# dkarpushkin/rs-pathtracing

Hardware: AMD Instinct MI355X
Metric: Msamples/sec cornell_box 1920x1080x256spp at 1/2/4/8 MI355X; RMS pixel delta (higher is better)
Workload: dtype f64; 1 GPU; cornell_box.json 1920x1080 256spp depth 8; config=c2, width=1920, height=1080, spp=256, depth=8, seed=1, parallelism=single GPU, wf_slots=2

## Files before the change

### __graft_entry__.py

```python
import importlib.util
import os
import subprocess
import sys
from pathlib import Path

ROOT = Path(__file__).resolve().parent


def load_package():
    if "rs_pathtracing_amd" in sys.modules:
        return sys.modules["rs_pathtracing_amd"]
    pkg = ROOT / "rs-pathtracing_amd"
    spec = importlib.util.spec_from_file_location("rs_pathtracing_amd", pkg / "__init__.py",
                                                  submodule_search_locations=[str(pkg)])
    mod = importlib.util.module_from_spec(spec)
    sys.modules["rs_pathtracing_amd"] = mod
    spec.loader.exec_module(mod)
    return mod


def build() -> None:
    env = dict(os.environ, PYTORCH_ROCM_ARCH="gfx950")
    jobs = str(min(8, os.cpu_count() or 1))
    subprocess.run(["make", "-j", jobs, "-C", str(ROOT / "rs-pathtracing_amd")], check=True, env=env)
    subprocess.run(["make", "-C", str(ROOT / "oracle")], check=True, env=env)
    subprocess.run(["make", "-j", jobs, "-C", str(ROOT / "tests" / "native")], check=True, env=env)
    subprocess.run(["make", "-C", str(ROOT / "tests" / "march_clip")], check=True, env=env)
    subprocess.run(["make", "-C", str(ROOT / "tools"), "pt_render"], check=True, env=env)
    pt = load_package()
    pt.lib()
    print("built", pt.LIB_PATH, "-", pt.version())


def smoke() -> None:
    import numpy as np

    pt = load_package()
    sys.path.insert(0, str(ROOT / "oracle"))
    import oracle

    text = (ROOT / "scenes" / "cornell_box.json").read_text()
    scene = pt.Scene.from_json(text, seed=1)
    r = pt.HipRenderer(scene, device=0, depth=8)
    w, h, spp = 48, 27, 2
    img = r.render(scene.camera(), pt.ImageParams(w, h), spp, seed=1)
    ref = oracle.Scene(text, seed=1).render(w, h, spp, 8, 1)
    rms = np.sqrt(np.mean((img - ref) ** 2, axis=0))
    exact = float(np.mean(np.all(img == ref, axis=1)))
    print("smoke: %dx%d@%dspp mean=%s rms=%s exact_pixels=%.4f" % (w, h, spp, img.mean(0), rms, exact))
    assert np.all(rms <= 1e-4), rms
# ... 8 lines not shown
```

### rs-pathtracing_amd/csrc/pt_api.cpp

```cpp
#include <hip/hip_runtime.h>

#include <algorithm>
#include <atomic>
#include <chrono>
#include <cmath>
#include <cstddef>
#include <cstring>
#include <new>
#include <string>
#include <thread>
#include <type_traits>
#include <vector>

#include "../../include/rs_pathtracing.h"
#include "pt_accel.hpp"
#include "pt_adaptive.hpp"
#include "pt_aov.hpp"
#include "pt_denoise.hpp"
#include "pt_kernel.hpp"
#include "pt_plan.hpp"
#include "pt_scene.hpp"
#include "pt_temporal.hpp"
#include "pt_tiles.hpp"
#include "pt_variance.hpp"
// ... 332 lines not shown
    const std::vector<DQGrid> qbuf = pack_qnodes(acc);
    hipError_t err = hipSetDevice(device);
    const DNodeC *nodes = upload(err, acc.cnodes, fault);
    const int32_t *leaf = upload(err, acc.leaf, fault);
    const int32_t *lin = upload(err, acc.lin, fault);
    const int32_t *march = upload(err, acc.march, fault);
    const DBox *boxes = upload(err, acc.boxes, fault);
    const DQGrid *qnodes = qbuf.empty() ? nullptr : upload(err, qbuf, fault);
    StagedAccel a{};
    view_set_accel(a, acc, nodes, qnodes, leaf, lin, march, boxes);
    if (err != hipSuccess) {
        free_staged(device, a);
        return hip_fail(err, "uploading the acceleration structure");
    }
    *out = a;
    return PT_OK;
}

int commit_accel(GpuShare &g, StagedAccel &a) {
    HIP_TRY(hipSetDevice(g.device));
    HIP_TRY(hipDeviceSynchronize());
    StagedAccel old = g.ds.view;
    view_set_accel(g.ds.view, a);
    a = StagedAccel{};
    free_staged(g.device, old);
    return PT_OK;
}

int init_share(GpuShare &g, int device, const Scene &S, const Accel &acc, const std::vector<DShape> &hs,
               const std::vector<DMaterial> &hm) {
    g.device = device;
    HIP_TRY(hipSetDevice(device));
    hipError_t err = hipStreamCreateWithFlags(&g.stream, hipStreamNonBlocking);
    const DShape *shapes = upload(err, hs);
    const DMaterial *mats = upload(err, hm);
    const bool tex = !S.textures.empty();
    const DTexture *textures = tex ? upload(err, S.textures) : nullptr;
    const DPerlin *perlins = tex ? upload(err, S.perlins) : nullptr;
    const DImage *images = tex ? upload(err, S.images) : nullptr;
    const uint8_t *pixels = tex ? upload(err, S.pixels) : nullptr;
    view_set_scene(g.ds.view, S, shapes, mats, textures, perlins, images, pixels);
    if (err == hipSuccess) err = hipEventCreateWithFlags(&g.shard_ev, hipEventDisableTiming);
    if (err == hipSuccess) err = hipMalloc((void **)&g.ds.view.guard, 4 * sizeof(unsigned long long));
    if (err == hipSuccess) err = hipMemset(g.ds.view.guard, 0, 4 * sizeof(unsigned long long));
    if (err != hipSuccess) return hip_fail(err, "uploading the scene");
    StagedAccel a{};
// ... 286 lines not shown
        r->fault_accel_alloc = (int)value;
        return PT_OK;
    }
    for (auto &g : r->gpus) {
        Tuning t = g.ws.tune;
        if (!tuning_set(&t, name, value))
            return fail(PT_ERR_INVALID, std::string("unknown option or value out of range: ") + name + " = " +
                                            std::to_string((long long)value));
        HIP_TRY(hipSetDevice(g.device));
        HIP_TRY(hipDeviceSynchronize());
        g.ws.tune = t;
        g.ds.view.diag = t.diag;
    }
    return PT_OK;
}

int pt_renderer_get_option(const pt_renderer *r, const char *name, int64_t *value) {
    if (!r || !name || !value) return fail(PT_ERR_INVALID, "null argument");
    if (!std::strcmp(name, "bvh_nodes")) {
        *value = r->gpus[0].ds.view.nnodes;
        return PT_OK;
    }
    if (ran_get(r->gpus[0].ws.ran, name, value)) return PT_OK;
    if (!tuning_get(r->gpus[0].ws.tune, name, value)) return fail(PT_ERR_INVALID, std::string("unknown option: ") + name);
    return PT_OK;
}

const char *pt_option_name(int index) {
    return index >= 0 && index < KNOB_COUNT ? KNOBS[index].name : nullptr;
}

int pt_renderer_peer_access(const pt_renderer *r, int *pairs, int *enabled) {
    if (!r) return fail(PT_ERR_INVALID, "null renderer");
    if (pairs) *pairs = r->peer_pairs;
    if (enabled) *enabled = r->peer_enabled;
    return PT_OK;
}

int pt_renderer_num_devices(const pt_renderer *r) { return r ? (int)r->gpus.size() : fail(PT_ERR_INVALID, "null renderer"); }

void pt_renderer_destroy(pt_renderer *r) {
    if (!r) return;
    if (r->started) (void)pt_render_stop(r);
    join_feeder(r);
    (void)sync_all(r);
    release_bands(r);
// ... 831 lines not shown
```

### rs-pathtracing_amd/csrc/pt_device.hpp

```cpp
#pragma once
#include <hip/hip_runtime.h>

#include <cstdint>

#include "pt_lprof.hpp"
#include "pt_march.hpp"
#include "pt_tiles.hpp"
#include "pt_torus.hpp"
#include "pt_types.hpp"

namespace pt {
namespace dev {

__device__ __forceinline__ bool stopped(const int *flag) {
    return flag && __hip_atomic_load(flag, __ATOMIC_RELAXED, __HIP_MEMORY_SCOPE_SYSTEM) != 0;
}

struct V3 {
    double x, y, z;
};
PT_HD V3 v3(double x, double y, double z) { return V3{x, y, z}; }
PT_HD V3 add(V3 a, V3 b) { return v3(a.x + b.x, a.y + b.y, a.z + b.z); }
PT_HD V3 sub(V3 a, V3 b) { return v3(a.x - b.x, a.y - b.y, a.z - b.z); }
PT_HD double dot(V3 a, V3 b) { return a.x * b.x + a.y * b.y + a.z * b.z; }
PT_HD V3 scale(V3 a, double s) { return v3(a.x * s, a.y * s, a.z * s); }
PT_HD V3 divs(V3 a, double s) { return v3(a.x / s, a.y / s, a.z / s); }
PT_HD V3 neg(V3 a) { return v3(-a.x, -a.y, -a.z); }
// ... 263 lines not shown

template <bool STATS>
PT_HD void bvh_leaf_test(const Scene &sc, const Ray &r, bool axis_ok, int first, int count, bool direct,
                         double min_t, double &best, int &who, Ctr *ct) {
    for (int k = 0; k < count; k++) {
        int i = direct ? first : sc.leaf[first + k];
        PT_LP(BVH_LEAF);
        double t;
        const DShape &S = sc.shapes[i];
        bool h;
        if (axis_ok && S.axis) {
            if (STATS) ct->c[C_TEST_SPHERE]++;
            h = sphere_axis_t(S.inv, r.o, r.d, min_t, best, &t);
        } else {
            h = shape_test<STATS, march::F_ANY, false>(S, r, min_t, best, &t, ct);
        }
        if (h && (t < best || i > who)) {
            best = t;
            who = i;
        }
    }
}

template <bool STATS = false, bool EXT = false, bool FMA_SLAB = false, bool QN = false, int PART = 3>
PT_HD void closest_nomarch(const Scene &sc, const Ray &r, V3 inv, double min_t, double *best_t, int *who_out,
                           Ctr *ct = nullptr, bool any = false) {
    double best = *best_t;
    int who = *who_out;
    double g_pz = 0.0, g_dz = 1.0, g_ox = 0.0, g_oy = 0.0, g_dx = 0.0, g_dy = 0.0;
    for (int k = 0; k < ((PART & 1) ? sc.nlin : 0); k++) {
        if (any && wave_all(who >= 0)) break;
        const int entry = uniform_index(uniform_load(&sc.lin[k]));
        const int i = entry & LIN_ID_MASK;
        const DShape s = uniform_shape(&sc.shapes[i]);
        PT_LP(ULIST_SHAPE);
        if (s.type == RECTANGLE) {
            if (STATS) ct->c[C_TEST_RECT]++;
            const double *m = s.inv;
            if (!(entry & LIN_GROUPED)) {
                g_pz = r.o.x * m[8] + r.o.y * m[9] + r.o.z * m[10];
                g_dz = r.d.x * m[8] + r.d.y * m[9] + r.d.z * m[10];
                g_ox = r.o.x * m[0] + r.o.y * m[1] + r.o.z * m[2];
                g_oy = r.o.x * m[4] + r.o.y * m[5] + r.o.z * m[6];
                g_dx = r.d.x * m[0] + r.d.y * m[1] + r.d.z * m[2];
                g_dy = r.d.x * m[4] + r.d.y * m[5] + r.d.z * m[6];
            }
            const double oz = g_pz + m[11];
            const double tt = -oz / g_dz;
            bool h = !(tt < min_t || tt > best);
            if (h) {
                PT_LP(RECT_ROWS);
                const double px = (g_ox + m[3]) + g_dx * tt, py = (g_oy + m[7]) + g_dy * tt;
                h = !(px < s.p[0] || px > s.p[2] || py < s.p[1] || py > s.p[3]);
            }
            if (h && (tt < best || i > who)) {
                best = tt;
                who = i;
            }
            continue;
        }
        if (s.type == CUBE || s.type == SPHERE) {
            if (STATS) ct->c[C_NODE_SLABS]++;
// ... 658 lines not shown
```

### rs-pathtracing_amd/csrc/pt_kernel.hip

```cpp
#include <hip/hip_runtime.h>

#include "pt_device.hpp"
#include "pt_kernel.hpp"

#include <cstdlib>
#include <cstring>

namespace pt {

using dev::Ray;
using dev::V3;

template <int NW, int WAVES, int FK = march::F_ANY>
__global__ __launch_bounds__(256, WAVES) void render_tiles(dev::Scene sc, FrameParams P, double *__restrict__ out) {
    if (P.stop) {
        __shared__ int halt;
        if (threadIdx.x == 0) {
            halt = dev::stopped(P.stop);
            if (halt) dev::note_stop(sc.guard, false);
        }
        __syncthreads();
        if (halt) return;
    }
    const uint32_t ti = P.tile_begin + blockIdx.x;
// ... 169 lines not shown
    if (l == (uint32_t)__ffsll((long long)bal) - 1) {
        atomicAdd(&acc[0], (unsigned long long)pt.trace);
        atomicAdd(&acc[1], (unsigned long long)pt.march);
        atomicAdd(&acc[2], (unsigned long long)pt.select);
        atomicAdd(&acc[3], (unsigned long long)(pt.finish + pt.scatter + pt.restart));
        atomicAdd(&acc[7], (unsigned long long)pt.finish);
        atomicAdd(&acc[8], (unsigned long long)pt.scatter);
        atomicAdd(&acc[9], (unsigned long long)pt.restart);
    }
    atomicAdd(&acc[4], (unsigned long long)pt.passes);
    atomicAdd(&acc[5], (unsigned long long)pt.march_passes);
    atomicMax(&acc[6], (unsigned long long)pt.passes);
}

#define PT_DISPATCH_NW(depth, CALL)                                        \
    switch (builds::stack_words(depth)) {                                  \
    case 4: { constexpr int NW = 4; CALL; } break;                         \
    case 8: { constexpr int NW = 8; CALL; } break;                         \
    case 16: { constexpr int NW = 16; CALL; } break;                       \
    default: { constexpr int NW = 32; CALL; } break;                       \
    }

hipError_t launch_render_wave(const dev::Scene &sc, const FrameParams &P, double *out, hipStream_t st,
                              WaveWorkspace *ws, const builds::Choice &ch, const uint32_t *tiles);

hipError_t launch_render(const DeviceScene &s, const FrameParams &P, double *out, hipStream_t st, WaveWorkspace &ws,
                         const uint32_t *tiles) {
    ws.ran = builds::Ran{};
    if (P.tile_count == 0) return hipSuccess;
    ws.refusal[0] = 0;
    builds::Inputs in{};
    in.ext = s.view.ext != 0;
    in.fkind = s.fkind;
    in.nnodes = s.view.nnodes;
    in.nmarch = s.view.nmarch;
    in.has_qnodes = s.view.qnodes != nullptr;
    in.scene_diag = s.view.diag;
    in.depth = P.depth;
    in.samples = (uint64_t)P.tile_count * TILE * TILE * P.spp;
    in.window = P.s_begin > 0 || (P.s_end && P.s_end < P.spp) || tiles != nullptr;
    in.window_empty = P.s_begin >= (P.s_end ? P.s_end : P.spp);
    in.wave_diag_on = PT_WAVE_DIAG && ws.diag;
    in.diag_buffer = ws.diag != nullptr;
    in.tune = ws.tune;
    const builds::Choice ch = builds::choose(in);
    if (ch.engine == builds::REFUSE) return hipErrorInvalidValue;
    if (ch.engine == builds::WAVE) return launch_render_wave(s.view, P, out, st, &ws, ch, tiles);
    if (tiles) return hipErrorInvalidValue;
    hipError_t e0 = timer_begin(ws.timer, st, K_MEGA);
    if (e0 != hipSuccess) return e0;
    bool launched = false;
#define X(NW, WAVES, FK)                                                             \
    if (ch.mega.is(NW, WAVES, FK)) {                                                 \
        render_tiles<NW, WAVES, FK><<<P.tile_count, 256, 0, st>>>(s.view, P, out);   \
        ws.ran.engine = builds::MEGA;                                                \
        ws.ran.mega = builds::key(NW, WAVES, FK);                                    \
        launched = true;                                                             \
    }
    PT_MEGA_BUILDS(X)
#undef X
    if (!launched) return hipErrorInvalidValue;
    e0 = hipGetLastError();
    if (e0 != hipSuccess) return e0;
    return timer_end(ws.timer, st);
}

hipError_t launch_unshard(const double *g, uint32_t width, uint32_t height, uint32_t world, double *frame,
                          hipStream_t st, uint32_t y0, uint32_t y1) {
    uint32_t tiles_x = (width + TILE - 1) / TILE, tiles_y = (height + TILE - 1) / TILE;
    uint32_t total = tiles_x * tiles_y;
// ... 96 lines not shown
```

### rs-pathtracing_amd/csrc/pt_kernel.hpp

```cpp
#pragma once
#include <hip/hip_runtime.h>

#include "../../include/rs_pathtracing.h"
#include "pt_builds.hpp"
#include "pt_types.hpp"

namespace pt {

struct DeviceScene {
    dev::Scene view = {};
    int nshapes = 0;
    int fkind = 0;
};

enum KernelKind : int { K_BOUNCE = 0, K_MARCH = 1, K_SELECT = 2, K_REDUCE = 3, K_MEGA = 4, K_UNWIND = 5, K_WALK = 6, K_KINDS = 7 };
struct KernelTimer;
KernelTimer *timer_new();
void timer_free(KernelTimer *t);
hipError_t timer_begin(KernelTimer *t, hipStream_t st, int kind);
hipError_t timer_end(KernelTimer *t, hipStream_t st);
hipError_t timer_collect(KernelTimer *t, double *ms, uint32_t *launches);

#ifndef PT_WAVE_DIAG
#define PT_WAVE_DIAG 0
#endif

struct WaveWorkspace {
    Tuning tune;
    void *base = nullptr;
    size_t bytes = 0;
    unsigned long long *diag = nullptr;
    KernelTimer *timer = nullptr;
    static constexpr int MAX_SLOTS = WF_MAX_SLOTS;
    hipStream_t side[MAX_SLOTS - 1] = {};
    hipEvent_t fork = nullptr, join[MAX_SLOTS - 1] = {}, reduced = nullptr;
    hipEvent_t done = nullptr;
    bool used = false;
    void *args_host = nullptr, *args_dev = nullptr;
    size_t args_bytes = 0;
    hipEvent_t args_ev = nullptr;
    bool args_pending = false;
    int device = -1;
    char refusal[320] = {};
    builds::Ran ran;
};
void wave_workspace_free(WaveWorkspace *ws);

hipError_t launch_render(const DeviceScene &s, const FrameParams &P, double *out, hipStream_t st, WaveWorkspace &ws,
                         const uint32_t *tiles = nullptr);
hipError_t launch_unshard(const double *gathered, uint32_t width, uint32_t height, uint32_t world, double *frame,
                          hipStream_t st, uint32_t y0 = 0, uint32_t y1 = ~0u);
hipError_t launch_encode_rgba8(const double *rgb, size_t p0, size_t p1, uint8_t *rgba, hipStream_t st);
hipError_t launch_closest_hit(const DeviceScene &s, const double *rays, size_t n, double min_t, double max_t,
                              pt_hit *out, hipStream_t st);
hipError_t launch_ray_color(const DeviceScene &s, const double *rays, uint64_t *states, size_t n, uint32_t depth,
                            double s11, double *out, hipStream_t st);
hipError_t launch_trace_pixels(const DeviceScene &s, const FrameParams &P, const uint32_t *pixels, size_t n,
                               double *out, hipStream_t st);

hipError_t launch_count_work(const DeviceScene &s, const FrameParams &P, const uint32_t *pixels, size_t n,
                             unsigned long long *ctr, hipStream_t st);

hipError_t launch_march_probe(const double *jobs, size_t n, double *t, int32_t *status, uint32_t *iters,
                              hipStream_t st);
hipError_t launch_render_timed(const DeviceScene &s, const FrameParams &P, double *out, unsigned long long *acc,
                               hipStream_t st);

}
```

### rs-pathtracing_amd/csrc/pt_lprof.hpp

```cpp
#pragma once
#include <hip/hip_runtime.h>

#ifdef PT_MARCH_REGIONS
namespace pt {
namespace mreg {
enum { R_ITER, R_POLY, R_PREFIX, R_HALVE, R_ADV, R_LIT, R_REFILL, R_TOTAL, R_N };
enum { P_iters, P_lin_init, P_lit_adds, P_advance_loops, P_evals, P_sir_inside, P_lin_fail_zero, P_lin_fail_q,
       P_lin_fail_tie, P_lin_fail_zone, P_N };
constexpr int G_N = 2 * R_N + 2 * P_N;
__device__ unsigned long long g_acc[G_N];
__shared__ unsigned long long t0[4][R_N], acc[4][R_N], accl[4][R_N], n0[4][R_N], pw[4][P_N], pl[4][P_N];
__device__ __forceinline__ unsigned long long now() {
    __builtin_amdgcn_sched_barrier(0);
    const unsigned long long t = __builtin_amdgcn_s_memtime();
    __builtin_amdgcn_sched_barrier(0);
    return t;
}
__device__ __forceinline__ bool leader() {
    const uint32_t lane = __builtin_amdgcn_mbcnt_hi(~0u, __builtin_amdgcn_mbcnt_lo(~0u, 0u));
    return lane == (uint32_t)__builtin_ctzll(__ballot(1));
}
__device__ __forceinline__ void begin(int r) {
    const unsigned long long m = __ballot(1);
    if (leader()) {
// ... 115 lines not shown
    const uint32_t lane = __builtin_amdgcn_mbcnt_hi(~0u, __builtin_amdgcn_mbcnt_lo(~0u, 0u));
    if (lane == (uint32_t)__builtin_ctzll(m)) {
        atomicAdd(&s_pass[k], 1ull);
        atomicAdd(&s_lanes[k], (unsigned long long)__popcll(m));
    }
}
__device__ __forceinline__ void begin_kernel() {
    if (threadIdx.x < N_POINTS) s_pass[threadIdx.x] = s_lanes[threadIdx.x] = 0;
    __syncthreads();
}
__device__ __forceinline__ void end_kernel() {
    __syncthreads();
    if (threadIdx.x < N_POINTS) {
        atomicAdd(&g_counts[threadIdx.x], s_pass[threadIdx.x]);
        atomicAdd(&g_counts[N_POINTS + threadIdx.x], s_lanes[threadIdx.x]);
    }
}
}
}
#endif
#if defined(PT_LANE_PROF) && defined(__HIP_DEVICE_COMPILE__)
#define PT_LP(k) pt::lprof::hit(pt::lprof::k)
#define PT_LP_BEGIN() pt::lprof::begin_kernel()
#define PT_LP_END() pt::lprof::end_kernel()
#else
#define PT_LP(k) ((void)0)
#define PT_LP_BEGIN() ((void)0)
#define PT_LP_END() ((void)0)
#endif
```

### rs-pathtracing_amd/csrc/pt_wave.hip

```cpp
#include <hip/hip_runtime.h>

#include <cstdio>
#include <cstdlib>
#include <cstring>
#include <vector>

#include "pt_lprof.hpp"

#include "pt_device.hpp"
#include "pt_kernel.hpp"
#include "pt_plan.hpp"

namespace pt {

using dev::MemStack;
using dev::Ray;
using dev::V3;

constexpr uint32_t WHO_MASK = (1u << 25) - 1u;
__host__ __device__ __forceinline__ uint32_t pack_who(int who, uint32_t count) {
    return (uint32_t)(who + 1) | (count << 25);
}
__host__ __device__ __forceinline__ int unpack_who(uint32_t w) { return (int)(w & WHO_MASK) - 1; }

// ... 9 lines not shown
    }
    __host__ __device__ uint32_t *d4(uint32_t k) const {
        return (uint32_t *)(base + (size_t)(k / BLK) * BLK_BYTES + 8 * 8 * BLK) + (k % BLK);
    }
    __host__ __device__ double &t(uint32_t k) const { return d8(k)[T * BLK]; }
    __host__ __device__ uint32_t &who(uint32_t k) const { return d4(k)[WHO * BLK]; }
};

struct WfView {
    PathSoA in, out;
    uint32_t *ids;
    double *att;
    double *leaf;
    uint8_t *status;
    uint32_t *list, *mq;
    double2 *jo;
    uint32_t *cnt;
    double *acc;
    uint32_t cap;
    uint32_t npix;
    uint32_t s0, ns;
    uint32_t tile0;
    const uint32_t *tile_map;
};

struct alignas(64) WfArgs {
    dev::Scene sc;
    FrameParams P;
    WfView v;
};

template <class T>
__device__ __forceinline__ const T &kargs(const T *p) {
    typedef const __attribute__((address_space(4))) T *cptr;
    cptr q = (cptr)p;
    asm volatile("" : "+s"(q));
    return *(const T *)q;
}

__device__ __forceinline__ uint32_t lane_id() {
    return __builtin_amdgcn_mbcnt_hi(~0u, __builtin_amdgcn_mbcnt_lo(~0u, 0u));
}

constexpr int UB = 4;
template <bool EXT>
__device__ __forceinline__ V3 unwind_mem(const dev::Scene &sc, MemStack &stk, V3 c) {
// ... 110 lines not shown
    PT_LP_BEGIN();
#define PT_BSTAMP(k)                                                \
    if (DIAG) {                                                     \
        __builtin_amdgcn_s_waitcnt(0);                              \
        const unsigned long long n_ = __builtin_amdgcn_s_memtime(); \
        dsec[k] += n_ - tst;                                        \
        tst = n_;                                                   \
    }
    for (uint32_t base = blockIdx.x * blockDim.x; base < count; base += stride) {
        if (DIAG) tst = __builtin_amdgcn_s_memtime();
        const WfArgs &a = kargs(A);
        const dev::Scene &sc = a.sc;
        const FrameParams &P = a.P;
        const WfView &v = a.v;
        const uint32_t i = base + threadIdx.x;
        bool live = i < count;
        uint32_t id = 0;
        Ray ray;
        dev::Rng rng{0};
        uint32_t depth = 0;
        MemStack stk{v.ids, (size_t)v.cap, 0, nullptr};
        int who = -1;
        double best = 0.0;
        if (live) {
            if (FIRST) {
                id = i;
                uint32_t x, y, sl, pl;
                slot_pixel(P, v, id, &x, &y, &sl, &pl);
                if (x >= P.width || y >= P.height || sl >= v.ns) {
                    live = false;
                } else {
                    rng.s = dev::sample_key(P.seed, (uint64_t)x + (uint64_t)y * P.width, v.s0 + sl);
                    ray = dev::camera_ray(P, x, y, rng);
                    depth = P.depth;
                    stk.base = v.ids + id;
                    if (EXT) stk.vb = v.att + id;
                }
            } else {
                const uint32_t p = v.list[i];
                PT_BSTAMP(0)
                uint32_t count;
                load_path(v.in, p, &id, &ray, &rng.s, P.depth + 1u - (uint32_t)it, &depth, &count, &who, &best);
                stk.base = v.ids + id;
                stk.n = DEEP ? (int)*deep_count(v, P.depth, id) : (int)count;
                if (EXT) stk.vb = v.att + id;
                PT_BSTAMP(1)
            }
        }
        bool need_march = false, long_job = false;
        V3 jo_o = dev::v3(0.0, 0.0, 0.0), jo_d = jo_o;
        double jo_st = 0.0, jo_en = 0.0;
        if (live) {
            PT_LP(LIVE);
            if (!FIRST) {
                V3 leaf;
                const bool ended = dev::shade<false, FK, EXT>(kargs(A).sc, who, best, ray, depth, stk, rng, P.s11, &leaf);
                PT_BSTAMP(2)
                if (ended) {
                    PT_LP(ENDED);
                    end_path(v, id, stk, leaf);
                    live = false;
                    PT_BSTAMP(3)
                }
            }
        }
        if (live && SPLIT) {
            best = __builtin_inf();
            who = -1;
        } else if (live) {
            PT_LP(TRACE);
            const V3 inv = dev::v3(1.0 / ray.d.x, 1.0 / ray.d.y, 1.0 / ray.d.z);
            best = __builtin_inf();
            who = -1;
            const bool any = depth == 0;
            dev::closest_nomarch<false, EXT, BIGBVH>(kargs(A).sc, ray, inv, T_MIN, &best, &who, nullptr, any);
            PT_BSTAMP(4)
            for (int k = 0; k < sc.nmarch && !need_march && !(any && who >= 0); k++) {
                const int s = dev::uniform_index(dev::uniform_load(&sc.march[k]));
                const DBox bx = dev::uniform_box(&sc.boxes[s]);
                if (!dev::slab(bx.lo, bx.hi, ray, inv, T_MIN, best)) continue;
                PT_LP(PRE_SLAB);
                const DShape S = dev::uniform_shape(&sc.shapes[s]);
                jo_o = dev::xf_point(S.inv, ray.o);
                jo_d = dev::xf_vector(S.inv, ray.d);
                need_march = march::shape_bound_k<FK>(dev::shape_params(S), jo_o.x, jo_o.y, jo_o.z, jo_d.x, jo_d.y,
                                                      jo_d.z, &jo_st, &jo_en);
                need_march = need_march && march::clip_to_best(best, S.p[0], &jo_st, &jo_en);
            }
            PT_BSTAMP(5)
            if (!need_march && dev::shade_decided(who, depth)) {
                if (any) PT_LP(ANY_END);
                else PT_LP(MISS_END);
                end_path(v, id, stk, dev::decided_leaf(who, ray));
                live = false;
            }
        }
        const uint32_t wbase = base + (threadIdx.x & ~63u);
        const uint64_t keep = __ballot(live);
        const uint32_t k = wbase + (uint32_t)__popcll(keep & ((1ull << (threadIdx.x & 63)) - 1ull));
        if (i < count && (threadIdx.x & 63) >= (uint32_t)__popcll(keep)) v.status[i] = 0u;
// ... 6 lines not shown
            __builtin_nontemporal_store((d2v){jo_d.y, jo_d.z}, j + 2);
            __builtin_nontemporal_store((d2v){jo_st, jo_en}, j + 3);
            const march::FParams F = dev::shape_params(dev::uniform_shape(&sc.shapes[dev::uniform_index(
                dev::uniform_load(&sc.march[0]))]));
            const V3 o = jo_o, d = jo_d;
            const double st = jo_st, en = jo_en;
            long_job = march::shape_f_k<FK>(F, o.x + d.x * st, o.y + d.y * st, o.z + d.z * st) < 0.0;
            const double dt = (en - st) * (1.0 / WF_PREDICT);
#pragma unroll
            for (int q = 0; q < WF_PREDICT; q++) {
                const double tq = st + dt * (q + 0.5);
                long_job = long_job || march::shape_f_k<FK>(F, o.x + d.x * tq, o.y + d.y * tq, o.z + d.z * tq) < 0.0;
            }
        }
        if (i < count) PT_LP(STORE);
        if (i < count && live) {
            store_path(v.out, k, id, ray, best, who, rng.s, DEEP ? 0u : (uint32_t)stk.n);
            if (DEEP) *deep_count(v, P.depth, id) = (uint32_t)stk.n;
            v.status[k] = live ? (need_march ? (long_job ? 7u : 3u) : 1u) : 0u;
        }
        PT_BSTAMP(6)
    }
#undef PT_BSTAMP
    PT_LP_END();
    if (DIAG && (threadIdx.x & 63) == 0)
        for (int k = 0; k < 7; k++) atomicAdd(&diag[36 + k], dsec[k]);
}


__device__ __forceinline__ void cp_bits(uint4 q, uint32_t *live, uint32_t *march, uint32_t *lng) {
    const uint32_t w[4] = {q.x, q.y, q.z, q.w};
    uint32_t l = 0, m = 0, g = 0;
#pragma unroll
    for (int k = 0; k < 4; k++) {
        l += __popc(w[k] & 0x01010101u);
        m += __popc(w[k] & 0x02020202u);
        g += __popc(w[k] & 0x04040404u);
    }
    *live = l;
    *march = m;
    *lng = g;
}

__device__ __forceinline__ uint32_t block_exscan(uint32_t x, uint32_t *total, uint32_t *lds ) {
    const uint32_t lane = threadIdx.x & 63, wv = threadIdx.x >> 6;
    uint32_t inc = x;
#pragma unroll
// ... 543 lines not shown
    if (ws->args_host) (void)hipHostFree(ws->args_host);
    if (ws->args_dev) (void)hipFree(ws->args_dev);
    ws->args_host = ws->args_dev = nullptr;
    ws->args_bytes = 0;
    ws->args_pending = false;
}

static void release_streams(WaveWorkspace *ws) {
    free_args(ws);
    for (int k = 0; k < WaveWorkspace::MAX_SLOTS - 1; k++) {
        if (ws->side[k]) (void)hipStreamDestroy(ws->side[k]);
        if (ws->join[k]) (void)hipEventDestroy(ws->join[k]);
        ws->side[k] = nullptr;
        ws->join[k] = nullptr;
    }
    if (ws->fork) (void)hipEventDestroy(ws->fork);
    if (ws->reduced) (void)hipEventDestroy(ws->reduced);
    if (ws->done) (void)hipEventDestroy(ws->done);
    if (ws->args_ev) (void)hipEventDestroy(ws->args_ev);
    ws->fork = ws->reduced = ws->done = ws->args_ev = nullptr;
    ws->used = false;
}

void wave_workspace_free(WaveWorkspace *ws) {
    release_streams(ws);
    timer_free(ws->timer);
    ws->timer = nullptr;
    if (ws->diag) (void)hipFree(ws->diag);
    ws->diag = nullptr;
    if (ws->base) (void)hipFree(ws->base);
    ws->base = nullptr;
    ws->bytes = 0;
}

static hipError_t reserve_args(WaveWorkspace *ws, size_t bytes) {
    hipError_t e;
    if (ws->args_pending) {
        if ((e = hipEventSynchronize(ws->args_ev)) != hipSuccess) return e;
        ws->args_pending = false;
    }
    if (bytes <= ws->args_bytes) return hipSuccess;
    if (ws->used && (e = hipEventSynchronize(ws->done)) != hipSuccess) return e;
    free_args(ws);
    if (bytes < ((size_t)64 << 10)) bytes = (size_t)64 << 10;
    if ((e = hipHostMalloc(&ws->args_host, bytes, hipHostMallocDefault)) != hipSuccess) {
        ws->args_host = nullptr;
        return e;
    }
    if ((e = hipMalloc(&ws->args_dev, bytes)) != hipSuccess) {
        ws->args_dev = nullptr;
        free_args(ws);
        return e;
// ... 92 lines not shown
    if (unwound)
        wf_reduce<EXT, true><<<blocks, 256, 0, st>>>(A, first, last, out);
    else
        wf_reduce<EXT, false><<<blocks, 256, 0, st>>>(A, first, last, out);
    return hipSuccess;
}

template <class F>
static hipError_t timed(KernelTimer *t, hipStream_t st, int kind, F launch) {
    hipError_t e = timer_begin(t, st, kind);
    if (e != hipSuccess) return e;
    if ((e = launch()) != hipSuccess) return e;
    if ((e = hipGetLastError()) != hipSuccess) return e;
    return timer_end(t, st);
}

static hipError_t ensure_streams(WaveWorkspace *ws, int slots) {
    int dev = 0;
    hipError_t e = hipGetDevice(&dev);
    if (e != hipSuccess) return e;
    if (ws->device != dev) {
        if (ws->used && ws->done && (e = hipEventSynchronize(ws->done)) != hipSuccess) return e;
        release_streams(ws);
        ws->device = dev;
    }
    if (!ws->fork && (e = hipEventCreateWithFlags(&ws->fork, hipEventDisableTiming)) != hipSuccess) return e;
    if (!ws->done && (e = hipEventCreateWithFlags(&ws->done, hipEventDisableTiming)) != hipSuccess) return e;
    if (!ws->reduced && (e = hipEventCreateWithFlags(&ws->reduced, hipEventDisableTiming)) != hipSuccess) return e;
    if (!ws->args_ev && (e = hipEventCreateWithFlags(&ws->args_ev, hipEventDisableTiming)) != hipSuccess) return e;
    for (int k = 0; k < slots - 1; k++) {
        if (!ws->side[k] && (e = hipStreamCreateWithFlags(&ws->side[k], hipStreamNonBlocking)) != hipSuccess) return e;
        if (!ws->join[k] && (e = hipEventCreateWithFlags(&ws->join[k], hipEventDisableTiming)) != hipSuccess) return e;
    }
    return hipSuccess;
}

struct Slot {
    WfView v;
    uint32_t *cp_blk;
    PathSoA set[2];
};

static hipStream_t slot_stream(const WaveWorkspace *ws, hipStream_t st, int j) { return j == 0 ? st : ws->side[j - 1]; }

hipError_t launch_render_wave(const dev::Scene &sc, const FrameParams &P0, double *out, hipStream_t st,
                              WaveWorkspace *ws, const builds::Choice &bc, const uint32_t *tiles) {
    if (P0.tile_count == 0 || P0.spp == 0) return hipSuccess;
    const Tuning &tu = ws->tune;
    plan::Input in;
    in.ntiles = P0.tile_count;
    in.s_begin = P0.s_begin;
    in.s_end = P0.s_end ? P0.s_end : P0.spp;
    in.spp = P0.spp;
    in.depth = P0.depth;
    in.progressive = P0.stop != nullptr;
    in.textured = sc.tex != nullptr;
    in.presel = bc.presel;
    in.wf_paths = tu.wf_paths;
    in.wf_slots = tu.wf_slots;
    in.wf_min_chunks = tu.wf_min_chunks;
    in.avail_bytes = plan::MEM_UNKNOWN;
    size_t free_b = 0, total_b = 0, hard_bytes = plan::MEM_UNKNOWN;
    if (hipMemGetInfo(&free_b, &total_b) == hipSuccess) {
        hard_bytes = free_b + ws->bytes;
        in.avail_bytes = hard_bytes > plan::RESERVE_BYTES ? hard_bytes - plan::RESERVE_BYTES : 0;
    }
    if (!plan::depth_ok(P0.depth)) {
        snprintf(ws->refusal, sizeof ws->refusal, "depth %u is above the largest supported depth, %u", P0.depth,
                 plan::MAX_DEPTH);
        return hipErrorInvalidValue;
    }
    const plan::Plan pl = plan::make_plan_fit(&in, hard_bytes);
    if (!plan::fits_device(pl, hard_bytes)) {
        snprintf(ws->refusal, sizeof ws->refusal,
                 "the wavefront workspace does not fit the device: depth %u, %s scene, %u paths per chunk on %d "
                 "stream(s) need %zu bytes, %zu bytes available",
                 P0.depth, in.textured ? "textured" : "untextured", pl.cap, pl.slots, pl.bytes, hard_bytes);
        return hipErrorOutOfMemory;
    }
    const plan::Layout &L = pl.lay;
    const std::vector<plan::Chunk> chunk_list = plan::chunk_list(in, pl);
    const int slots = pl.slots, iters = pl.iters;
    const uint32_t s_begin = in.s_begin, s_end = in.s_end;

    hipError_t e = ensure_streams(ws, slots);
    if (e != hipSuccess) return e;
    if (ws->used && (e = hipStreamWaitEvent(st, ws->done, 0)) != hipSuccess) return e;
    if ((e = reserve(ws, pl.bytes)) != hipSuccess) return e;
    Slot sl[WaveWorkspace::MAX_SLOTS];
    for (int k = 0; k < slots; k++) {
        char *slot = (char *)ws->base + (size_t)k * L.slot_stride;
        auto at = [&](plan::Region r) { return L.size[r] ? (void *)(slot + L.off[r]) : nullptr; };
        sl[k].set[0] = PathSoA{(char *)at(plan::R_SET0), pl.cap};
        sl[k].set[1] = PathSoA{(char *)at(plan::R_SET1), pl.cap};
        sl[k].cp_blk = (uint32_t *)at(plan::R_CP_BLK);
        WfView &v = sl[k].v;
        v.ids = (uint32_t *)at(plan::R_IDS);
        v.leaf = (double *)at(plan::R_LEAF);
        v.list = (uint32_t *)at(plan::R_LIST);
        v.mq = (uint32_t *)at(plan::R_MQ);
        v.status = (uint8_t *)at(plan::R_STATUS);
        v.cnt = (uint32_t *)at(plan::R_CNT);
        v.att = (double *)at(plan::R_ATT);
        v.jo = (double2 *)at(plan::R_JO);
        v.acc = (double *)((char *)ws->base + L.acc);
        v.cap = pl.cap;
    }

    const uint32_t march_slice = (uint32_t)tu.wf_march_slice;
    unsigned long long *const bounce_diag = bc.bounce.diag ? ws->diag : nullptr;
    unsigned long long *const march_diag = bc.march.diag ? ws->diag : nullptr;
    const size_t nargs = chunk_list.size() * 2;
    const size_t list_off = (nargs * sizeof(WfArgs) + 15) & ~(size_t)15;
    const size_t args_bytes = tiles ? list_off + (size_t)P0.tile_count * sizeof(uint32_t) : nargs * sizeof(WfArgs);
    if ((e = reserve_args(ws, args_bytes)) != hipSuccess) return e;
    WfArgs *ah = (WfArgs *)ws->args_host, *ad = (WfArgs *)ws->args_dev;
    const uint32_t *tile_map = nullptr;
    if (tiles) {
        memcpy((char *)ws->args_host + list_off, tiles, (size_t)P0.tile_count * sizeof(uint32_t));
        tile_map = (const uint32_t *)((char *)ws->args_dev + list_off);
    }
    for (size_t ci = 0; ci < chunk_list.size(); ci++) {
        const plan::Chunk &ch = chunk_list[ci];
        const int j = ch.slot;
        WfView v = sl[j].v;
        v.tile0 = P0.tile_begin + ch.g0;
        v.tile_map = tile_map;
        v.npix = ch.gt * TILE * TILE;
        v.s0 = ch.s0;
        v.ns = ch.ns;
        for (int h = 0; h < 2; h++) {
            v.in = sl[j].set[h];
            v.out = sl[j].set[h ^ 1];
            ah[2 * ci + h] = WfArgs{sc, P0, v};
        }
    }
    if ((e = hipMemcpyAsync(ad, ah, args_bytes, hipMemcpyHostToDevice, st)) != hipSuccess) return e;
    if ((e = hipEventRecord(ws->args_ev, st)) != hipSuccess) return e;
    ws->args_pending = true;
    if (slots > 1) {
        if ((e = hipEventRecord(ws->fork, st)) != hipSuccess) return e;
        for (int k = 0; k < slots - 1; k++)
            if ((e = hipStreamWaitEvent(ws->side[k], ws->fork, 0)) != hipSuccess) return e;
    }
    for (size_t r0 = 0; r0 < chunk_list.size();) {
        size_t r1 = r0;
        while (r1 < chunk_list.size() && chunk_list[r1].step == chunk_list[r0].step) r1++;
        for (size_t c = r0; c < r1; c++) {
            const int j = chunk_list[c].slot;
            const hipStream_t cs = slot_stream(ws, st, j);
// ... 105 lines not shown
```

Before: 2322 Msamples/s.

## Cull unreachable shapes for primary rays using per-8x8-block frustum masks

Adds a per-frame table, built by a small kernel, that holds a 64-bit mask for each 8x8 pixel block. Each bit says whether a list shape or march shape's bounding box can intersect that block's sub-frustum. The first-bounce kernel reads the mask with a wave-uniform load and skips shapes outside the frustum in both the linear list and the march loop. Grouped-rectangle caching is made aware of skipped entries. The table is cached by camera key and accel generation, at the cost of an extra kernel launch when the camera changes and some added branching in the primary-ray loop.

```diff
diff --git a/__graft_entry__.py b/__graft_entry__.py
--- a/__graft_entry__.py
+++ b/__graft_entry__.py
@@ -26,6 +26,7 @@
     subprocess.run(["make", "-C", str(ROOT / "oracle")], check=True, env=env)
     subprocess.run(["make", "-j", jobs, "-C", str(ROOT / "tests" / "native")], check=True, env=env)
     subprocess.run(["make", "-C", str(ROOT / "tests" / "march_clip")], check=True, env=env)
+    subprocess.run(["make", "-C", str(ROOT / "tests" / "first_cull")], check=True, env=env)
     subprocess.run(["make", "-C", str(ROOT / "tools"), "pt_render"], check=True, env=env)
     pt = load_package()
     pt.lib()
diff --git a/rs-pathtracing_amd/csrc/pt_api.cpp b/rs-pathtracing_amd/csrc/pt_api.cpp
--- a/rs-pathtracing_amd/csrc/pt_api.cpp
+++ b/rs-pathtracing_amd/csrc/pt_api.cpp
@@ -378,6 +378,7 @@
     HIP_TRY(hipDeviceSynchronize());
     StagedAccel old = g.ds.view;
     view_set_accel(g.ds.view, a);
+    g.ds.accel_gen++;
     a = StagedAccel{};
     free_staged(g.device, old);
     return PT_OK;
@@ -710,6 +711,11 @@
         return PT_OK;
     }
     if (ran_get(r->gpus[0].ws.ran, name, value)) return PT_OK;
+    if (!std::strcmp(name, "first_cull_bits")) {
+        HIP_TRY(hipSetDevice(r->gpus[0].device));
+        HIP_TRY(first_cull_bits(r->gpus[0].ws, value));
+        return PT_OK;
+    }
     if (!tuning_get(r->gpus[0].ws.tune, name, value)) return fail(PT_ERR_INVALID, std::string("unknown option: ") + name);
     return PT_OK;
 }
diff --git a/rs-pathtracing_amd/csrc/pt_cull.hpp b/rs-pathtracing_amd/csrc/pt_cull.hpp
--- /dev/null
+++ b/rs-pathtracing_amd/csrc/pt_cull.hpp
@@ -0,0 +1,115 @@
+#pragma once
+#ifdef __HIPCC__
+#include <hip/hip_runtime.h>
+#endif
+
+#include <cmath>
+#include <cstdint>
+
+#include "pt_dims.hpp"
+#include "pt_types.hpp"
+
+namespace pt {
+namespace cull {
+
+constexpr uint32_t BLOCK = 8;
+constexpr int LIST_BITS = 32;
+constexpr uint64_t ALL = ~0ull;
+constexpr double EPS = 1e-9;
+constexpr double MIN_COS = 1e-6;
+
+PT_HD uint32_t blocks_across(uint32_t pixels) { return (pixels + BLOCK - 1) / BLOCK; }
+
+struct Plane {
+    double x, y, z;
+};
+PT_HD double pdot(const Plane &n, double vx, double vy, double vz, double *mag) {
+    const double a = n.x * vx, b = n.y * vy, c = n.z * vz;
+    *mag = fabs(a) + fabs(b) + fabs(c);
+    return a + b + c;
+}
+PT_HD bool finite3(double x, double y, double z) {
+    const double s = x + y + z;
+    return s - s == 0.0;
+}
+
+PT_HD uint64_t first_cull_mask(const FrameParams &P, const int32_t *lin, int nlin, const int32_t *march, int nmarch,
+                               const DBox *boxes, uint32_t bx, uint32_t by) {
+    if (!(P.pixel_resolution > 0.0)) return ALL;
+    const double px[4] = {(double)(BLOCK * bx) - 1.0, (double)(BLOCK * bx + BLOCK) + 1.0,
+                          (double)(BLOCK * bx + BLOCK) + 1.0, (double)(BLOCK * bx) - 1.0};
+    const double py[4] = {(double)(BLOCK * by) - 1.0, (double)(BLOCK * by) - 1.0, (double)(BLOCK * by + BLOCK) + 1.0,
+                          (double)(BLOCK * by + BLOCK) + 1.0};
+    double c[4][3], axis[3];
+    const double ax = P.pixel_resolution * (0.5 * (double)P.width), ay = P.pixel_resolution * (0.5 * (double)P.height);
+    for (int a = 0; a < 3; a++) axis[a] = ((P.left_top[a] + P.right[a] * ax) - P.up[a] * ay) - P.pos[a];
+    const double aa = axis[0] * axis[0] + axis[1] * axis[1] + axis[2] * axis[2];
+    for (int j = 0; j < 4; j++) {
+        const double sx = P.pixel_resolution * px[j], sy = P.pixel_resolution * py[j];
+        for (int a = 0; a < 3; a++) c[j][a] = ((P.left_top[a] + P.right[a] * sx) - P.up[a] * sy) - P.pos[a];
+        if (!finite3(c[j][0], c[j][1], c[j][2])) return ALL;
+        const double ca = c[j][0] * axis[0] + c[j][1] * axis[1] + c[j][2] * axis[2];
+        const double cc = c[j][0] * c[j][0] + c[j][1] * c[j][1] + c[j][2] * c[j][2];
+        if (!(ca > 0.0 && ca * ca > (MIN_COS * MIN_COS) * (cc * aa))) return ALL;
+    }
+    const double mid[3] = {(c[0][0] + c[1][0]) + (c[2][0] + c[3][0]), (c[0][1] + c[1][1]) + (c[2][1] + c[3][1]),
+                           (c[0][2] + c[1][2]) + (c[2][2] + c[3][2])};
+    Plane n[4];
+    for (int j = 0; j < 4; j++) {
+        const double *u = c[j], *w = c[(j + 1) & 3];
+        Plane q{u[1] * w[2] - u[2] * w[1], u[2] * w[0] - u[0] * w[2], u[0] * w[1] - u[1] * w[0]};
+        double mag;
+        if (pdot(q, mid[0], mid[1], mid[2], &mag) < 0.0) q = Plane{-q.x, -q.y, -q.z};
+        if (!finite3(q.x, q.y, q.z)) return ALL;
+        n[j] = q;
+        for (int i = 0; i < 4; i++) {
+            const double d = pdot(q, c[i][0], c[i][1], c[i][2], &mag);
+            const bool on = i == j || i == ((j + 1) & 3);
+            if (on ? !(d >= -EPS * mag) : !(d > EPS * mag)) return ALL;
+        }
+    }
+    auto reachable = [&](int shape, bool *ok) {
+        const DBox &b = boxes[shape];
+        if (!finite3(b.lo[0], b.lo[1], b.lo[2]) || !finite3(b.hi[0], b.hi[1], b.hi[2])) {
+            *ok = false;
+            return true;
+        }
+        for (int j = 0; j < 4; j++) {
+            bool all_out = true;
+            for (int k = 0; k < 8 && all_out; k++) {
+                const double vx = ((k & 1) ? b.hi[0] : b.lo[0]) - P.pos[0];
+                const double vy = ((k & 2) ? b.hi[1] : b.lo[1]) - P.pos[1];
+                const double vz = ((k & 4) ? b.hi[2] : b.lo[2]) - P.pos[2];
+                double mag;
+                const double d = pdot(n[j], vx, vy, vz, &mag);
+                all_out = d < -EPS * mag;
+            }
+            if (all_out) return false;
+        }
+        return true;
+    };
+    uint64_t mask = 0;
+    bool ok = true;
+    for (int k = 0; k < nlin && k < LIST_BITS; k++)
+        if (reachable(lin[k] & LIN_ID_MASK, &ok)) mask |= 1ull << k;
+    for (int k = 0; k < nmarch && k < 64 - LIST_BITS; k++)
+        if (reachable(march[k], &ok)) mask |= 1ull << (LIST_BITS + k);
+    return ok ? mask : ALL;
+}
+
+struct CasterKey {
+    double pos[3], right[3], up[3], left_top[3], pixel_resolution;
+    uint32_t width, height;
+};
+inline CasterKey caster_key(const FrameParams &P) {
+    CasterKey k;
+    for (int a = 0; a < 3; a++) k.pos[a] = P.pos[a], k.right[a] = P.right[a], k.up[a] = P.up[a], k.left_top[a] = P.left_top[a];
+    k.pixel_resolution = P.pixel_resolution;
+    k.width = P.width;
+    k.height = P.height;
+    return k;
+}
+static_assert(sizeof(CasterKey) == 13 * 8 + 8, "CasterKey is compared bytewise: no padding");
+
+}
+}
diff --git a/rs-pathtracing_amd/csrc/pt_device.hpp b/rs-pathtracing_amd/csrc/pt_device.hpp
--- a/rs-pathtracing_amd/csrc/pt_device.hpp
+++ b/rs-pathtracing_amd/csrc/pt_device.hpp
@@ -3,6 +3,7 @@
 
 #include <cstdint>
 
+#include "pt_cull.hpp"
 #include "pt_lprof.hpp"
 #include "pt_march.hpp"
 #include "pt_tiles.hpp"
@@ -312,22 +313,29 @@
     }
 }
 
-template <bool STATS = false, bool EXT = false, bool FMA_SLAB = false, bool QN = false, int PART = 3>
+template <bool STATS = false, bool EXT = false, bool FMA_SLAB = false, bool QN = false, int PART = 3,
+          bool CULL = false>
 PT_HD void closest_nomarch(const Scene &sc, const Ray &r, V3 inv, double min_t, double *best_t, int *who_out,
-                           Ctr *ct = nullptr, bool any = false) {
+                           Ctr *ct = nullptr, bool any = false, uint64_t cull_mask = ~0ull) {
     double best = *best_t;
     int who = *who_out;
     double g_pz = 0.0, g_dz = 1.0, g_ox = 0.0, g_oy = 0.0, g_dx = 0.0, g_dy = 0.0;
+    bool g_valid = false;
     for (int k = 0; k < ((PART & 1) ? sc.nlin : 0); k++) {
         if (any && wave_all(who >= 0)) break;
         const int entry = uniform_index(uniform_load(&sc.lin[k]));
         const int i = entry & LIN_ID_MASK;
+        if (CULL) {
+            if (!(entry & LIN_GROUPED)) g_valid = false;
+            if (k < cull::LIST_BITS && !((cull_mask >> k) & 1ull)) continue;
+        }
         const DShape s = uniform_shape(&sc.shapes[i]);
         PT_LP(ULIST_SHAPE);
         if (s.type == RECTANGLE) {
             if (STATS) ct->c[C_TEST_RECT]++;
             const double *m = s.inv;
-            if (!(entry & LIN_GROUPED)) {
+            if (CULL ? !g_valid : !(entry & LIN_GROUPED)) {
+                g_valid = true;
                 g_pz = r.o.x * m[8] + r.o.y * m[9] + r.o.z * m[10];
                 g_dz = r.d.x * m[8] + r.d.y * m[9] + r.d.z * m[10];
                 g_ox = r.o.x * m[0] + r.o.y * m[1] + r.o.z * m[2];
diff --git a/rs-pathtracing_amd/csrc/pt_kernel.hip b/rs-pathtracing_amd/csrc/pt_kernel.hip
--- a/rs-pathtracing_amd/csrc/pt_kernel.hip
+++ b/rs-pathtracing_amd/csrc/pt_kernel.hip
@@ -215,11 +215,12 @@
     }
 
 hipError_t launch_render_wave(const dev::Scene &sc, const FrameParams &P, double *out, hipStream_t st,
-                              WaveWorkspace *ws, const builds::Choice &ch, const uint32_t *tiles);
+                              WaveWorkspace *ws, const builds::Choice &ch, const uint32_t *tiles, uint64_t accel_gen);
 
 hipError_t launch_render(const DeviceScene &s, const FrameParams &P, double *out, hipStream_t st, WaveWorkspace &ws,
                          const uint32_t *tiles) {
     ws.ran = builds::Ran{};
+    ws.first_cull.used = false;
     if (P.tile_count == 0) return hipSuccess;
     ws.refusal[0] = 0;
     builds::Inputs in{};
@@ -238,7 +239,7 @@
     in.tune = ws.tune;
     const builds::Choice ch = builds::choose(in);
     if (ch.engine == builds::REFUSE) return hipErrorInvalidValue;
-    if (ch.engine == builds::WAVE) return launch_render_wave(s.view, P, out, st, &ws, ch, tiles);
+    if (ch.engine == builds::WAVE) return launch_render_wave(s.view, P, out, st, &ws, ch, tiles, s.accel_gen);
     if (tiles) return hipErrorInvalidValue;
     hipError_t e0 = timer_begin(ws.timer, st, K_MEGA);
     if (e0 != hipSuccess) return e0;
diff --git a/rs-pathtracing_amd/csrc/pt_kernel.hpp b/rs-pathtracing_amd/csrc/pt_kernel.hpp
--- a/rs-pathtracing_amd/csrc/pt_kernel.hpp
+++ b/rs-pathtracing_amd/csrc/pt_kernel.hpp
@@ -3,6 +3,7 @@
 
 #include "../../include/rs_pathtracing.h"
 #include "pt_builds.hpp"
+#include "pt_cull.hpp"
 #include "pt_types.hpp"
 
 namespace pt {
@@ -11,6 +12,7 @@
     dev::Scene view = {};
     int nshapes = 0;
     int fkind = 0;
+    uint64_t accel_gen = 0;
 };
 
 enum KernelKind : int { K_BOUNCE = 0, K_MARCH = 1, K_SELECT = 2, K_REDUCE = 3, K_MEGA = 4, K_UNWIND = 5, K_WALK = 6, K_KINDS = 7 };
@@ -43,8 +45,19 @@
     int device = -1;
     char refusal[320] = {};
     builds::Ran ran;
+    struct FirstCull {
+        uint64_t *table = nullptr;
+        size_t cap = 0;
+        size_t blocks = 0;
+        bool valid = false;
+        cull::CasterKey key = {};
+        uint64_t accel_gen = 0;
+        const void *boxes = nullptr;
+        bool used = false;
+    } first_cull;
 };
 void wave_workspace_free(WaveWorkspace *ws);
+hipError_t first_cull_bits(const WaveWorkspace &ws, int64_t *bits);
 
 hipError_t launch_render(const DeviceScene &s, const FrameParams &P, double *out, hipStream_t st, WaveWorkspace &ws,
                          const uint32_t *tiles = nullptr);
diff --git a/rs-pathtracing_amd/csrc/pt_lprof.hpp b/rs-pathtracing_amd/csrc/pt_lprof.hpp
--- a/rs-pathtracing_amd/csrc/pt_lprof.hpp
+++ b/rs-pathtracing_amd/csrc/pt_lprof.hpp
@@ -161,9 +161,16 @@
 #if defined(PT_LANE_PROF) && defined(__HIP_DEVICE_COMPILE__)
 #define PT_LP(k) pt::lprof::hit(pt::lprof::k)
 #define PT_LP_BEGIN() pt::lprof::begin_kernel()
-#define PT_LP_END() pt::lprof::end_kernel()
+#ifdef PT_LANE_PROF_IT
+#define PT_LP_END(it)                                      \
+    do {                                                   \
+        if ((it) == PT_LANE_PROF_IT) pt::lprof::end_kernel(); \
+    } while (0)
+#else
+#define PT_LP_END(it) pt::lprof::end_kernel()
+#endif
 #else
 #define PT_LP(k) ((void)0)
 #define PT_LP_BEGIN() ((void)0)
-#define PT_LP_END() ((void)0)
+#define PT_LP_END(it) ((void)0)
 #endif
diff --git a/rs-pathtracing_amd/csrc/pt_wave.hip b/rs-pathtracing_amd/csrc/pt_wave.hip
--- a/rs-pathtracing_amd/csrc/pt_wave.hip
+++ b/rs-pathtracing_amd/csrc/pt_wave.hip
@@ -55,6 +55,7 @@
     uint32_t s0, ns;
     uint32_t tile0;
     const uint32_t *tile_map;
+    const uint64_t *cull;
 };
 
 struct alignas(64) WfArgs {
@@ -211,10 +212,11 @@
         MemStack stk{v.ids, (size_t)v.cap, 0, nullptr};
         int who = -1;
         double best = 0.0;
+        uint32_t x = 0, y = 0;
         if (live) {
             if (FIRST) {
                 id = i;
-                uint32_t x, y, sl, pl;
+                uint32_t sl, pl;
                 slot_pixel(P, v, id, &x, &y, &sl, &pl);
                 if (x >= P.width || y >= P.height || sl >= v.ns) {
                     live = false;
@@ -236,6 +238,16 @@
                 PT_BSTAMP(1)
             }
         }
+        uint64_t cull_mask = ~0ull;
+        if (FIRST && !SPLIT) {
+            if (const uint64_t *tab = v.cull) {
+                const uint32_t bx = __builtin_amdgcn_readfirstlane(x / cull::BLOCK);
+                const uint32_t by = __builtin_amdgcn_readfirstlane(y / cull::BLOCK);
+                const uint32_t nbx = cull::blocks_across(P.width), nby = cull::blocks_across(P.height);
+                typedef const __attribute__((address_space(4))) uint64_t *ctab;
+                if (bx < nbx && by < nby) cull_mask = ((ctab)tab)[(size_t)by * nbx + bx];
+            }
+        }
         bool need_march = false, long_job = false;
         V3 jo_o = dev::v3(0.0, 0.0, 0.0), jo_d = jo_o;
         double jo_st = 0.0, jo_en = 0.0;
@@ -262,9 +274,11 @@
             best = __builtin_inf();
             who = -1;
             const bool any = depth == 0;
-            dev::closest_nomarch<false, EXT, BIGBVH>(kargs(A).sc, ray, inv, T_MIN, &best, &who, nullptr, any);
+            dev::closest_nomarch<false, EXT, BIGBVH, false, 3, FIRST>(kargs(A).sc, ray, inv, T_MIN, &best, &who, nullptr,
+                                                                     any, cull_mask);
             PT_BSTAMP(4)
             for (int k = 0; k < sc.nmarch && !need_march && !(any && who >= 0); k++) {
+                if (FIRST && k < 64 - cull::LIST_BITS && !((cull_mask >> (cull::LIST_BITS + k)) & 1ull)) continue;
                 const int s = dev::uniform_index(dev::uniform_load(&sc.march[k]));
                 const DBox bx = dev::uniform_box(&sc.boxes[s]);
                 if (!dev::slab(bx.lo, bx.hi, ray, inv, T_MIN, best)) continue;
@@ -317,7 +331,7 @@
         PT_BSTAMP(6)
     }
 #undef PT_BSTAMP
-    PT_LP_END();
+    PT_LP_END(it);
     if (DIAG && (threadIdx.x & 63) == 0)
         for (int k = 0; k < 7; k++) atomicAdd(&diag[36 + k], dsec[k]);
 }
@@ -907,12 +921,18 @@
     ws->used = false;
 }
 
+static void free_cull(WaveWorkspace *ws) {
+    if (ws->first_cull.table) (void)hipFree(ws->first_cull.table);
+    ws->first_cull = WaveWorkspace::FirstCull{};
+}
+
 void wave_workspace_free(WaveWorkspace *ws) {
     release_streams(ws);
     timer_free(ws->timer);
     ws->timer = nullptr;
     if (ws->diag) (void)hipFree(ws->diag);
     ws->diag = nullptr;
+    free_cull(ws);
     if (ws->base) (void)hipFree(ws->base);
     ws->base = nullptr;
     ws->bytes = 0;
@@ -1051,6 +1071,7 @@
     if (ws->device != dev) {
         if (ws->used && ws->done && (e = hipEventSynchronize(ws->done)) != hipSuccess) return e;
         release_streams(ws);
+        free_cull(ws);
         ws->device = dev;
     }
     if (!ws->fork && (e = hipEventCreateWithFlags(&ws->fork, hipEventDisableTiming)) != hipSuccess) return e;
@@ -1072,8 +1093,71 @@
 
 static hipStream_t slot_stream(const WaveWorkspace *ws, hipStream_t st, int j) { return j == 0 ? st : ws->side[j - 1]; }
 
+static __global__ __launch_bounds__(256) void wf_cull_table(FrameParams P, const int32_t *__restrict__ lin, int nlin,
+                                                            const int32_t *__restrict__ march, int nmarch,
+                                                            const DBox *__restrict__ boxes, uint32_t nbx, uint32_t nby,
+                                                            uint64_t *__restrict__ table) {
+    const uint32_t b = blockIdx.x * blockDim.x + threadIdx.x;
+    if (b >= nbx * nby) return;
+    table[b] = cull::first_cull_mask(P, lin, nlin, march, nmarch, boxes, b % nbx, b / nbx);
+}
+
+static hipError_t first_cull_table(WaveWorkspace *ws, const dev::Scene &sc, uint64_t accel_gen, const FrameParams &P,
+                                   const builds::Choice &bc, hipStream_t st, const uint64_t **table) {
+    *table = nullptr;
+    if (bc.bounce.split || (sc.nlin == 0 && sc.nmarch == 0)) return hipSuccess;
+    WaveWorkspace::FirstCull &fc = ws->first_cull;
+    const cull::CasterKey key = cull::caster_key(P);
+    const uint32_t nbx = cull::blocks_across(P.width), nby = cull::blocks_across(P.height);
+    const size_t blocks = (size_t)nbx * nby;
+    if (blocks == 0 || blocks > 0xffffffffu) return hipSuccess;
+    fc.used = true;
+    *table = fc.table;
+    if (fc.valid && fc.accel_gen == accel_gen && fc.boxes == sc.boxes && fc.blocks == blocks &&
+        !memcmp(&fc.key, &key, sizeof key))
+        return hipSuccess;
+    fc.valid = false;
+    hipError_t e;
+    if (blocks > fc.cap) {
+        if (fc.table) (void)hipFree(fc.table);
+        fc.table = nullptr;
+        fc.cap = 0;
+        *table = nullptr;
+        if ((e = hipMalloc((void **)&fc.table, blocks * sizeof(uint64_t))) != hipSuccess) {
+            fc.table = nullptr;
+            fc.used = false;
+            return e;
+        }
+        fc.cap = blocks;
+    }
+    wf_cull_table<<<(uint32_t)((blocks + 255) / 256), 256, 0, st>>>(P, sc.lin, sc.nlin, sc.march, sc.nmarch, sc.boxes,
+                                                                    nbx, nby, fc.table);
+    if ((e = hipGetLastError()) != hipSuccess) return e;
+    fc.key = key;
+    fc.accel_gen = accel_gen;
+    fc.boxes = sc.boxes;
+    fc.blocks = blocks;
+    fc.valid = true;
+    *table = fc.table;
+    return hipSuccess;
+}
+
+hipError_t first_cull_bits(const WaveWorkspace &ws, int64_t *bits) {
+    *bits = -1;
+    const WaveWorkspace::FirstCull &fc = ws.first_cull;
+    if (!fc.used || !fc.valid || !fc.table) return hipSuccess;
+    hipError_t e;
+    if (ws.used && (e = hipEventSynchronize(ws.done)) != hipSuccess) return e;
+    std::vector<uint64_t> h(fc.blocks);
+    if ((e = hipMemcpy(h.data(), fc.table, fc.blocks * sizeof(uint64_t), hipMemcpyDeviceToHost)) != hipSuccess) return e;
+    int64_t n = 0;
+    for (uint64_t m : h) n += __builtin_popcountll(m);
+    *bits = n;
+    return hipSuccess;
+}
+
 hipError_t launch_render_wave(const dev::Scene &sc, const FrameParams &P0, double *out, hipStream_t st,
-                              WaveWorkspace *ws, const builds::Choice &bc, const uint32_t *tiles) {
+                              WaveWorkspace *ws, const builds::Choice &bc, const uint32_t *tiles, uint64_t accel_gen) {
     if (P0.tile_count == 0 || P0.spp == 0) return hipSuccess;
     const Tuning &tu = ws->tune;
     plan::Input in;
@@ -1116,6 +1200,8 @@
     if (e != hipSuccess) return e;
     if (ws->used && (e = hipStreamWaitEvent(st, ws->done, 0)) != hipSuccess) return e;
     if ((e = reserve(ws, pl.bytes)) != hipSuccess) return e;
+    const uint64_t *cull_table = nullptr;
+    if ((e = first_cull_table(ws, sc, accel_gen, P0, bc, st, &cull_table)) != hipSuccess) return e;
     Slot sl[WaveWorkspace::MAX_SLOTS];
     for (int k = 0; k < slots; k++) {
         char *slot = (char *)ws->base + (size_t)k * L.slot_stride;
@@ -1155,6 +1241,7 @@
         WfView v = sl[j].v;
         v.tile0 = P0.tile_begin + ch.g0;
         v.tile_map = tile_map;
+        v.cull = cull_table;
         v.npix = ch.gt * TILE * TILE;
         v.s0 = ch.s0;
         v.ns = ch.ns;
```

After: 2362 Msamples/s, median of 6. +1.7%, better.
